# ajzhai/PEANUT

Measured on AMD Instinct MI355X. Metric: maps/sec for 480x480x(4+N_cat) prediction fwd, batch 32, higher is better.
Workload: dtype f32; 1 GPU; 480x480, 14-channel (4+10) partial maps -> 6-class prediction forward (PSPNet R50-V1c-D8), batch 32 per GPU, seeded random-init weights; survey_config=2, global_batch=32, parallelism=dp1 (map shards, no data-path collective)

## Files before the change

peanut_amd/csrc/options.h:

```cpp
#pragma once
#include <stdlib.h>
#include <string.h>

#include <string>

namespace peanut {

enum OptionId {
  OPT_PW_GLDS, OPT_PW256_MINK, OPT_PW256_MINTILES, OPT_PW256_PHASE, OPT_PW256_SKIP_PAD, OPT_PW256W_MINK, OPT_PW256W_MINTILES, OPT_PW256P_MINK, OPT_PW256P_MINTILES, OPT_PW256P_FLUSH, OPT_PW256P_ORDER, OPT_PW256P_STREAMK, OPT_PW256WP_MINK, OPT_PW256WP_MINTILES, OPT_PW256WP_NPRE, OPT_PW256WP_STAGGER, OPT_PW_ARES, OPT_PW_SKINNY,
  OPT_PW_ARES_MINUNITS, OPT_PATCH_MINTILES, OPT_STEM_NCHW, OPT_BN64_MAXK, OPT_PW_BN64_MAXK, OPT_PW64_MAXTILES, OPT_FP32_BK, OPT_NCHUNK, OPT_RES_PREFETCH, OPT_SPLIT_MODEL,
  OPT_RS_CONV, OPT_RS_BN64_MAXK, OPT_RS256_MINK, OPT_RS256_MINTILES, OPT_RS64_MAXK, OPT_RS64_MAXTILES,
  OPT_WINO_M, OPT_WINO_HEAD_M, OPT_WINO6_MAXDIL, OPT_WINO5_MINDIL, OPT_WINO_FLUSH_CH, OPT_WINO_MIN_CIN, OPT_WINO_NARROW_MINPIX, OPT_WINO_SMALL_MAXWG, OPT_DEFER_SPLITK,
  OPT_PPM_OVERLAP, OPT_PPM_GROUPED, OPT_PPM_TERM_ROWS, OPT_PPM_GROUP_ROWS, OPT_RCNN_WINO_M, OPT_RCNN_STEM_S2D, OPT_RCNN_RPN_FUSED, OPT_RCNN_FPN_OVERLAP, OPT_RCNN_RANK_SORT, OPT_RCNN_TOPK_SLICE, OPT_RCNN_NMS_LEVELS, OPT_FMM_LOCAL32, OPT_FMM_MAX_PASSES, OPT_FMM_BLOCKED, OPT_FMM_INNER,
  OPT_DEBUG_POISON_ALLOC,
  OPT_COUNT
};

struct OptionInfo {
  const char* key;
  long long def;
  bool upload_time;
  const char* help;
};

inline const OptionInfo* option_table() {
  static const OptionInfo t[OPT_COUNT] = {
      {"pw_glds", 1, false, "fp32 1x1 convs / grouped GEMMs on the LDS-DMA kernels of conv_pw.hip (0: conv_igemm)"},
      {"pw256_mink", 1024, false, "fewest input channels for the 256 x 128 three-stage kernel"},
      {"pw256_mintiles", 256, false, "fewest 256 x 128 tiles for that kernel"},
      {"pw256_phase", 1, false, "the two waves of a SIMD request their LDS-DMA pieces half an iteration apart"},
      {"pw256_skip_pad", 1, false, "256 x 128 kernel, grouped GEMMs: waves whose rows are all group padding issue no MFMAs (0: compute the zero rows)"},
      {"pw256w_mink", 768, false, "fewest input channels for the 256 x 256 two-stage kernel (0: off)"},
      {"pw256w_mintiles", 1536, false, "fewest 256 x 256 tiles for that kernel"},
      {"pw256p_mink", 512, false, "fewest input channels for the persistent 256 x 128 kernel (conv_pw256p.hip; 0: off)"},
      {"pw256p_mintiles", 512, false, "fewest 256 x 128 tiles for that kernel"},
// ... 10 lines not shown
      {"patch_mintiles", 1024, false, "3x3 convs of 16 / 32 input channels on the persistent LDS-patch kernel (conv_patch.hip) from this many 8 x 16 output tiles (0: off)"},
      {"stem_nchw", 1, false, "prediction forward: the first stem conv reads the NCHW input itself (conv_patch.hip, NCHW variant) instead of a layout pass + NHWC conv (fp32 mode, when the patch kernel takes the layer)"},
      {"bn64_maxk", 256, true, "128 x 64 tiles for layers with at most this many input channels"},
      {"pw_bn64_maxk", 128, true, "pointwise layers / Winograd position GEMMs: weights PACKED 64 wide up to this many input channels (wider layers: 128-wide packing, 64-wide tiles chosen per shape)"},
      {"pw64_maxtiles", 512, false, "a 128-wide-packed pointwise layer with at most bn64_maxk input channels runs 128 x 64 tiles while its 128 x 128 tiling has fewer tiles than this (two per CU)"},
      {"fp32_bk", 0, true, "16: force 16-channel k-tiles in conv_igemm (experiment)"},
      {"nchunk", 8, false, "n-tiles per chunk of the tile order (0: n fastest over all n-tiles)"},
      {"res_prefetch", 1, false, "request the first residual rows before the last k-tile's MFMAs"},
      {"split_model", 1, false, "tail split-K plan counts CUs (1) or resident slots (0)"},
      {"rs_conv", 1, true, "emulated modes: non-pointwise convs on conv_rs.hip (0: fp32 MFMA kernel)"},
      {"rs_bn64_maxk", 128, true, "emulated modes: 128 x 64 tiles up to this many input channels"},
      {"rs256_mink", 512, false, "emulated modes: fewest input channels for the 256 x 256 kernel"},
      {"rs256_mintiles", 256, false, "emulated modes: fewest 256 x 256 tiles for it"},
      {"rs64_maxk", 512, false, "emulated modes: 64 x 64 tiles up to this many input channels"},
      {"rs64_maxtiles", 128, false, "emulated modes: ... and below this many 128-row tiles"},
      {"wino_m", 0, true, "4 / 5 / 6: force one Winograd form on every eligible layer (0: policy)"},
      {"wino_head_m", 0, true, "4 / 5 / 6: Winograd form of the PSP bottleneck (0: policy)"},
      {"wino6_maxdil", 4, true, "largest dilation that gets an F(6x6) form"},
      {"wino5_mindil", 4, true, "smallest dilation that also gets an F(5x5) form (0: none)"},
      {"wino_flush_ch", 64, true, "channels per partial sum of the position GEMMs' two-level accumulation (0: off)"},
      {"wino_min_cin", 0, true, "fewest input channels of a Winograd layer (0: the planner's policy)"},
      {"wino_narrow_minpix", 20000, false, "layers under 128 channels take their Winograd form from this many input pixels on (round 6: 100 000 -> 20 000 -- with the small-problem transforms one 720 x 720 map's layer1 conv2, 32 400 pixels, gains 5 us per layer as F(6x6); profiles/r9e)"},
      {"wino_small_maxwg", 1024, false, "Winograd transforms: launches with fewer workgroups than this of the one-thread-per-tile kernels take the small-problem variants (a workgroup per tile and 64-channel slice, a thread per line, through LDS; bit-identical; 0: never)"},
      {"defer_splitk", 1, false, "a Bottleneck conv1 whose every tile is split along k leaves its partial tiles unsummed and conv2's (small-problem) Winograd input transform sums them: one launch fewer per block at batch 1, bit-identical (0: every conv runs its own reduce); read when a (B, H, W) plan is built"},
      {"ppm_overlap", -1, false, "pyramid branch of the PSP head on a side stream: 0 / 1, -1 = by size"},
      {"ppm_grouped", -1, false, "per-scale PSP GEMMs as one grouped launch: 0 / 1, -1 = by size"},
      {"ppm_term_rows", 1, false, "folded pyramid term: one wave per output row, no barrier in the row loop (0: the workgroup-wide two-phase kernel)"},
      {"ppm_group_rows", 0, false, "pyramid pooling, row pass: rows added up per workgroup (1..5; 0 = by size: as many as still leave ~768 workgroups)"},
      {"rcnn_wino_m", 0, true, "detector front end: 4 / 5 / 6 pins one Winograd form (0: per shape)"},
      {"rcnn_stem_s2d", 1, true, "detector stem 7x7 stride 2 as a space-to-depth 4x4 conv"},
      {"rcnn_rpn_fused", 1, false, "detector: the RPN head on all five pyramid levels as one chain (five input transforms, ONE grouped Winograd GEMM, five output transforms, one objectness and one anchor-delta GEMM over all levels' rows: 12 launches instead of 25); read when a (B, H, W) plan is built"},
      {"rcnn_fpn_overlap", 0, false, "detector: the FPN output convs of p5, p4, p3 on a side stream next to the lateral / top-down chain that ends in p2's (round 5 experiment, bit-identical; measured SLOWER at batch 1, 5.70 against 5.61 ms per frame, profiles/r8: off); read when a (B, H, W) plan is built"},
      {"rcnn_rank_sort", 1, false, "detector: the RPN candidates of an image are ordered by counting the larger keys (n / 64 workgroups) instead of one workgroup's bitonic sort (round 5; same order: the keys are distinct)"},
      {"rcnn_topk_slice", 20480, false, "detector: objectness logits per workgroup of the per-level top-k (a level is cut into up to 8 ranges whose k largest are merged by counting; 0: one workgroup per level, round 4)"},
      {"rcnn_nms_levels", 1, false, "detector: the proposal NMS level by level (five 16 x 16-word suppression blocks and five scans per image side by side, post-NMS top-k by counting) instead of one score-sorted list per image (round 5; same proposals)"},
      {"fmm_local32", 1, false, "goal solver: single-precision local solve inside a tile"},
      {"fmm_max_passes", 24, false, "goal solver: hard ceiling of the second-order ordering passes; they stop as soon as a pass changes nothing (6-10 passes on the agent's 960 x 960 map; peanut_goal_converged reports whether they reached their fixed point)"},
      {"fmm_blocked", 1, false, "goal solver: a wave relaxes its 8 x 8 block of the tile to convergence between workgroup barriers (round 5; 0: one Jacobi sweep of the whole tile per barrier pair)"},
      {"fmm_inner", 48, false, "goal solver: iterations a wave spends on its block before it publishes it (blocked rounds)"},
      {"debug_poison_alloc", 0, false, "test switch: every device allocation the library makes for itself (workspace arenas, conv / Winograd / split-K scratch, the detector's and the goal solver's buffers, the map projection's arrays, uploaded weights before their copy) is filled with 0xFF bytes straight after hipMalloc -- fp32 / fp64 read NaN, int reads -1, 64-bit keys all ones -- so a kernel that reads a slot nothing wrote shows up as a changed result (tests/test_workspace_gpu.py); 0: allocations stay as the allocator returns them, no extra call"},
  };
  return t;
}

struct Options {
  long long v[OPT_COUNT];
// ... 49 lines not shown
```

peanut_amd/csrc/winograd.hip:

```cpp
#include <stdlib.h>

#include <atomic>

#include "common.h"
#include "conv_common.h"

namespace peanut {

namespace {

template <typename V>
__device__ __forceinline__ V fmak(V a, float k, V c) { return __builtin_elementwise_fma(a, (V)k, c); }

__device__ __forceinline__ void bt6(const f32x4 d0, const f32x4 d1, const f32x4 d2, const f32x4 d3, const f32x4 d4,
                                    const f32x4 d5, f32x4& t0, f32x4& t1, f32x4& t2, f32x4& t3, f32x4& t4, f32x4& t5) {
#pragma clang fp contract(off)
  const f32x4 a = fmak(d2, -2.25f, d4), b = fmak(d3, 0.75f, -1.6875f * d1);
  const f32x4 c = fmak(d2, -0.5625f, d4), e = fmak(d3, 1.5f, -0.84375f * d1);
  t0 = fmak(d0, 1.265625f, fmak(d2, -2.8125f, d4));
  t1 = a + b;
  t2 = a - b;
  t3 = c + e;
  t4 = c - e;
  t5 = fmak(d1, 1.265625f, fmak(d3, -2.8125f, d5));
}

__device__ __forceinline__ void at6(const f32x4 m0, const f32x4 m1, const f32x4 m2, const f32x4 m3, const f32x4 m4,
                                    const f32x4 m5, f32x4& y0, f32x4& y1, f32x4& y2, f32x4& y3) {
#pragma clang fp contract(off)
  const f32x4 s12 = m1 + m2, d12 = m1 - m2, s34 = m3 + m4, d34 = m3 - m4;
  y0 = m0 + s12 + s34;
  y1 = fmak(d12, 0.75f, 1.5f * d34);
  y2 = fmak(s12, 0.5625f, 2.25f * s34);
  y3 = fmak(d12, 0.421875f, fmak(d34, 3.375f, m5));
}

struct WinoGeom {
  int B, H, W, C;
  int d, th, tw;
  long long n_tiles, m_pad;
};

__device__ __forceinline__ void decode_tile(const WinoGeom& g, long long t, int& b, int& oy, int& ox, int& ty, int& tx) {
  tx = (int)(t % g.tw); t /= g.tw;
  ty = (int)(t % g.th); t /= g.th;
  ox = (int)(t % g.d); t /= g.d;
  oy = (int)(t % g.d);
  b = (int)(t / g.d);
}

__device__ __forceinline__ bool decode_thread(long long idx, int groups, long long n_tiles, int& cg, long long& tile) {
  cg = (int)(idx % groups);
  tile = idx / groups;
  return tile < n_tiles;
}

__global__ __launch_bounds__(256) void wino_input_kernel(const float* __restrict__ x, float* __restrict__ V, const WinoGeom g) {
  const int groups = g.C >> 2;
  const long long total = g.n_tiles * groups;
  for (long long idx = (long long)blockIdx.x * blockDim.x + threadIdx.x; idx < total;
       idx += (long long)gridDim.x * blockDim.x) {
    int cg;
    long long tile;
    if (!decode_thread(idx, groups, g.n_tiles, cg, tile)) continue;
    int b, oy, ox, ty, tx;
    decode_tile(g, tile, b, oy, ox, ty, tx);
    const int r0 = oy + g.d * (4 * ty - 1), c0 = ox + g.d * (4 * tx - 1);
    const float* xb = x + (size_t)b * g.H * g.W * g.C + cg * 4;
    f32x4 p[6][6];
#pragma unroll
    for (int i = 0; i < 6; ++i) {
      const int r = r0 + i * g.d;
      const bool rok = (unsigned)r < (unsigned)g.H;
#pragma unroll
      for (int j = 0; j < 6; ++j) {
        const int c = c0 + j * g.d;
        f32x4 v = {0.f, 0.f, 0.f, 0.f};
        if (rok && (unsigned)c < (unsigned)g.W) v = *reinterpret_cast<const f32x4*>(xb + ((size_t)r * g.W + c) * g.C);
        p[i][j] = v;
      }
    }
#pragma unroll
    for (int j = 0; j < 6; ++j)
      bt6(p[0][j], p[1][j], p[2][j], p[3][j], p[4][j], p[5][j], p[0][j], p[1][j], p[2][j], p[3][j], p[4][j], p[5][j]);
    float* vb = V + (size_t)tile * g.C + cg * 4;
    const size_t pos_stride = (size_t)g.m_pad * g.C;
#pragma unroll
    for (int i = 0; i < 6; ++i) {
      f32x4 t0, t1, t2, t3, t4, t5;
      bt6(p[i][0], p[i][1], p[i][2], p[i][3], p[i][4], p[i][5], t0, t1, t2, t3, t4, t5);
      float* o = vb + (size_t)(i * 6) * pos_stride;
      *reinterpret_cast<f32x4*>(o) = t0;
      *reinterpret_cast<f32x4*>(o + pos_stride) = t1;
      *reinterpret_cast<f32x4*>(o + 2 * pos_stride) = t2;
      *reinterpret_cast<f32x4*>(o + 3 * pos_stride) = t3;
      *reinterpret_cast<f32x4*>(o + 4 * pos_stride) = t4;
      *reinterpret_cast<f32x4*>(o + 5 * pos_stride) = t5;
    }
  }
}

template <bool RES>
__global__ __launch_bounds__(256) void wino_output_kernel(const float* __restrict__ Mb, const float* __restrict__ scale,
                                                          const float* __restrict__ shift, const float* __restrict__ res,
                                                          float* __restrict__ y, const WinoGeom g, int relu) {
  const int groups = g.C >> 2;
  const long long total = g.n_tiles * groups;
  for (long long idx = (long long)blockIdx.x * blockDim.x + threadIdx.x; idx < total;
       idx += (long long)gridDim.x * blockDim.x) {
    int ng;
    long long tile;
    if (!decode_thread(idx, groups, g.n_tiles, ng, tile)) continue;
    int b, oy, ox, ty, tx;
    decode_tile(g, tile, b, oy, ox, ty, tx);
    const int r0 = oy + g.d * 4 * ty, c0 = ox + g.d * 4 * tx;
    if (r0 >= g.H || c0 >= g.W) continue;
    const float* mb = Mb + (size_t)tile * g.C + ng * 4;
    const size_t pos_stride = (size_t)g.m_pad * g.C;
    f32x4 q[6][4];
#pragma unroll
    for (int i = 0; i < 6; ++i) {
      const float* s = mb + (size_t)(i * 6) * pos_stride;
      const f32x4 m0 = __builtin_nontemporal_load(reinterpret_cast<const f32x4*>(s));
      const f32x4 m1 = __builtin_nontemporal_load(reinterpret_cast<const f32x4*>(s + pos_stride));
      const f32x4 m2 = __builtin_nontemporal_load(reinterpret_cast<const f32x4*>(s + 2 * pos_stride));
      const f32x4 m3 = __builtin_nontemporal_load(reinterpret_cast<const f32x4*>(s + 3 * pos_stride));
      const f32x4 m4 = __builtin_nontemporal_load(reinterpret_cast<const f32x4*>(s + 4 * pos_stride));
      const f32x4 m5 = __builtin_nontemporal_load(reinterpret_cast<const f32x4*>(s + 5 * pos_stride));
      at6(m0, m1, m2, m3, m4, m5, q[i][0], q[i][1], q[i][2], q[i][3]);
    }
    const f32x4 sc = *reinterpret_cast<const f32x4*>(scale + ng * 4);
    const f32x4 sh = *reinterpret_cast<const f32x4*>(shift + ng * 4);
    const size_t img = (size_t)b * g.H * g.W;
    f32x4 rn[4];
    auto res_column = [&](int j, f32x4 (&dst)[4]) __attribute__((always_inline)) {
// ... 16 lines not shown
        if (j + 1 < 4) res_column(j + 1, rn);
      }
      f32x4 o0, o1, o2, o3;
      at6(q[0][j], q[1][j], q[2][j], q[3][j], q[4][j], q[5][j], o0, o1, o2, o3);
      const int c = c0 + j * g.d;
      if (c >= g.W) continue;
      const f32x4 o[4] = {o0, o1, o2, o3};
#pragma unroll
      for (int a = 0; a < 4; ++a) {
        const int r = r0 + a * g.d;
        if (r >= g.H) continue;
        const size_t off = (img + (size_t)r * g.W + c) * g.C + ng * 4;
        f32x4 v = o[a] * sc + sh;
        if constexpr (RES) v += rc[a];
        if (relu) v = relu_keep_nan(v);
        *reinterpret_cast<f32x4*>(y + off) = v;
      }
    }
  }
}

typedef float f32x2 __attribute__((ext_vector_type(2)));

__device__ __forceinline__ void bt8(const f32x2 d0, const f32x2 d1, const f32x2 d2, const f32x2 d3, const f32x2 d4, const f32x2 d5,
                                    const f32x2 d6, const f32x2 d7, f32x2& t0, f32x2& t1, f32x2& t2, f32x2& t3, f32x2& t4,
                                    f32x2& t5, f32x2& t6, f32x2& t7) {
#pragma clang fp contract(off)
  const f32x2 e1 = 4.f * d2 + fmak(d4, -5.f, d6), o1 = 2.f * d1 + fmak(d3, -2.5f, 0.5f * d5);
  const f32x2 e2 = fmak(d4, -4.25f, d2) + d6, o2 = fmak(d3, -4.25f, d1) + d5;
  const f32x2 e3 = 0.25f * d2 + fmak(d4, -1.25f, d6), o3 = 0.5f * d1 + fmak(d3, -2.5f, 2.f * d5);
  const f32x2 r0 = fmak(d2 - d4, 5.25f, d6 - d0), r7 = fmak(d3 - d5, 5.25f, d7 - d1);
  t0 = r0; t1 = e1 + o1; t2 = e1 - o1; t3 = e2 + o2; t4 = e2 - o2; t5 = e3 + o3; t6 = e3 - o3; t7 = r7;
}

__device__ __forceinline__ void at8(const f32x2 m0, const f32x2 m1, const f32x2 m2, const f32x2 m3, const f32x2 m4, const f32x2 m5,
                                    const f32x2 m6, const f32x2 m7, f32x2& y0, f32x2& y1, f32x2& y2, f32x2& y3, f32x2& y4, f32x2& y5) {
#pragma clang fp contract(off)
  const f32x2 s1 = m1 + m2, d1 = m1 - m2, s2 = m3 + m4, d2 = m3 - m4, s3 = m5 + m6, d3 = m5 - m6;
  y0 = m0 + s1 + s2 + s3;
  y1 = 0.5f * d1 + d2 + 2.f * d3;
  y2 = 0.25f * s1 + s2 + 4.f * s3;
  y3 = 0.125f * d1 + d2 + 8.f * d3;
  y4 = 0.0625f * s1 + s2 + 16.f * s3;
  y5 = 0.03125f * d1 + d2 + 32.f * d3 + m7;
}

__global__ __launch_bounds__(256) void wino6_input_kernel(const float* __restrict__ x, float* __restrict__ V, const WinoGeom g) {
  const int groups = g.C >> 1;
  const long long total = g.n_tiles * groups;
  for (long long idx = (long long)blockIdx.x * blockDim.x + threadIdx.x; idx < total;
       idx += (long long)gridDim.x * blockDim.x) {
    int cg;
    long long tile;
    if (!decode_thread(idx, groups, g.n_tiles, cg, tile)) continue;
    int b, oy, ox, ty, tx;
    decode_tile(g, tile, b, oy, ox, ty, tx);
    const int r0 = oy + g.d * (6 * ty - 1), c0 = ox + g.d * (6 * tx - 1);
    const float* xb = x + (size_t)b * g.H * g.W * g.C + cg * 2;
    f32x2 p[8][8];
#pragma unroll
    for (int i = 0; i < 8; ++i) {
      const int r = r0 + i * g.d;
      const bool rok = (unsigned)r < (unsigned)g.H;
#pragma unroll
      for (int j = 0; j < 8; ++j) {
        const int c = c0 + j * g.d;
        f32x2 v = {0.f, 0.f};
        if (rok && (unsigned)c < (unsigned)g.W) v = *reinterpret_cast<const f32x2*>(xb + ((size_t)r * g.W + c) * g.C);
        p[i][j] = v;
      }
    }
#pragma unroll
    for (int j = 0; j < 8; ++j)
      bt8(p[0][j], p[1][j], p[2][j], p[3][j], p[4][j], p[5][j], p[6][j], p[7][j],
          p[0][j], p[1][j], p[2][j], p[3][j], p[4][j], p[5][j], p[6][j], p[7][j]);
    float* vb = V + (size_t)tile * g.C + cg * 2;
    const size_t pos_stride = (size_t)g.m_pad * g.C;
#pragma unroll
    for (int i = 0; i < 8; ++i) {
      f32x2 t[8];
      bt8(p[i][0], p[i][1], p[i][2], p[i][3], p[i][4], p[i][5], p[i][6], p[i][7], t[0], t[1], t[2], t[3], t[4], t[5], t[6], t[7]);
      float* o = vb + (size_t)(i * 8) * pos_stride;
#pragma unroll
      for (int j = 0; j < 8; ++j) *reinterpret_cast<f32x2*>(o + j * pos_stride) = t[j];
    }
  }
}

template <bool RES>
__global__ __launch_bounds__(256) void wino6_output_kernel(const float* __restrict__ Mb, const float* __restrict__ scale,
                                                           const float* __restrict__ shift, const float* __restrict__ res,
                                                           float* __restrict__ y, const WinoGeom g, int relu) {
  const int groups = g.C >> 1;
  const long long total = g.n_tiles * groups;
  for (long long idx = (long long)blockIdx.x * blockDim.x + threadIdx.x; idx < total;
       idx += (long long)gridDim.x * blockDim.x) {
    int ng;
    long long tile;
    if (!decode_thread(idx, groups, g.n_tiles, ng, tile)) continue;
    int b, oy, ox, ty, tx;
    decode_tile(g, tile, b, oy, ox, ty, tx);
    const int r0 = oy + g.d * 6 * ty, c0 = ox + g.d * 6 * tx;
    if (r0 >= g.H || c0 >= g.W) continue;
    const float* mb = Mb + (size_t)tile * g.C + ng * 2;
    const size_t pos_stride = (size_t)g.m_pad * g.C;
    f32x2 q[8][6];
#pragma unroll
    for (int i = 0; i < 8; ++i) {
      const float* s = mb + (size_t)(i * 8) * pos_stride;
      f32x2 m[8];
#pragma unroll
      for (int j = 0; j < 8; ++j) m[j] = __builtin_nontemporal_load(reinterpret_cast<const f32x2*>(s + j * pos_stride));
      at8(m[0], m[1], m[2], m[3], m[4], m[5], m[6], m[7], q[i][0], q[i][1], q[i][2], q[i][3], q[i][4], q[i][5]);
    }
    const f32x2 sc = *reinterpret_cast<const f32x2*>(scale + ng * 2);
    const f32x2 sh = *reinterpret_cast<const f32x2*>(shift + ng * 2);
    const size_t img = (size_t)b * g.H * g.W;
    f32x2 rn[6];
    auto res_column = [&](int j, f32x2 (&dst)[6]) __attribute__((always_inline)) {
      const int c = c0 + j * g.d;
#pragma unroll
      for (int a = 0; a < 6; ++a) {
// ... 7 lines not shown
#pragma unroll
    for (int j = 0; j < 6; ++j) {
      f32x2 rc[6];
      if constexpr (RES) {
#pragma unroll
        for (int a = 0; a < 6; ++a) rc[a] = rn[a];
        if (j + 1 < 6) res_column(j + 1, rn);
      }
      f32x2 o[6];
      at8(q[0][j], q[1][j], q[2][j], q[3][j], q[4][j], q[5][j], q[6][j], q[7][j], o[0], o[1], o[2], o[3], o[4], o[5]);
      const int c = c0 + j * g.d;
      if (c >= g.W) continue;
#pragma unroll
      for (int a = 0; a < 6; ++a) {
        const int r = r0 + a * g.d;
        if (r >= g.H) continue;
        const size_t off = (img + (size_t)r * g.W + c) * g.C + ng * 2;
        f32x2 v = o[a] * sc + sh;
        if constexpr (RES) v += rc[a];
        if (relu) { v.x = relu_keep_nan(v.x); v.y = relu_keep_nan(v.y); }
        *reinterpret_cast<f32x2*>(y + off) = v;
      }
    }
  }
}

__device__ __forceinline__ void bt7(const f32x2 d0, const f32x2 d1, const f32x2 d2, const f32x2 d3, const f32x2 d4, const f32x2 d5,
                                    const f32x2 d6, f32x2& t0, f32x2& t1, f32x2& t2, f32x2& t3, f32x2& t4, f32x2& t5, f32x2& t6) {
  const f32x2 r0 = d5 - 0.75f * d0 + 0.25f * d1 + 3.75f * d2 - 1.25f * d3 - 3.f * d4;
  const f32x2 r1 = d5 + 1.5f * d1 + 2.5f * (d2 - d3 - d4);
  const f32x2 r2 = d5 - 1.5f * d1 + 3.5f * (d2 - d4) + 0.5f * d3;
  const f32x2 r3 = d5 + 0.75f * d1 + 0.5f * d2 - 3.25f * d3 - 2.f * d4;
  const f32x2 r4 = d5 - 0.75f * d1 + d2 + 2.75f * d3 - 4.f * d4;
  const f32x2 r5 = d5 + 0.25f * d1 - 1.25f * d3;
  const f32x2 r6 = d6 - 0.75f * d1 + 0.25f * d2 + 3.75f * d3 - 1.25f * d4 - 3.f * d5;
  t0 = r0; t1 = r1; t2 = r2; t3 = r3; t4 = r4; t5 = r5; t6 = r6;
}

__device__ __forceinline__ void at7(const f32x2 m0, const f32x2 m1, const f32x2 m2, const f32x2 m3, const f32x2 m4, const f32x2 m5,
                                    const f32x2 m6, f32x2& y0, f32x2& y1, f32x2& y2, f32x2& y3, f32x2& y4) {
  const f32x2 s1 = m1 + m2, d1 = m1 - m2, s2 = m3 + m4, d2 = m3 - m4;
  y0 = m0 + s1 + s2 + m5;
  y1 = 0.5f * d1 + d2 + 3.f * m5;
  y2 = 0.25f * s1 + s2 + 9.f * m5;
  y3 = 0.125f * d1 + d2 + 27.f * m5;
  y4 = 0.0625f * s1 + s2 + 81.f * m5 + m6;
}

__global__ __launch_bounds__(256) void wino5_input_kernel(const float* __restrict__ x, float* __restrict__ V, const WinoGeom g) {
  const int groups = g.C >> 1;
  const long long total = g.n_tiles * groups;
  for (long long idx = (long long)blockIdx.x * blockDim.x + threadIdx.x; idx < total;
       idx += (long long)gridDim.x * blockDim.x) {
    int cg;
    long long tile;
    if (!decode_thread(idx, groups, g.n_tiles, cg, tile)) continue;
    int b, oy, ox, ty, tx;
    decode_tile(g, tile, b, oy, ox, ty, tx);
    const int r0 = oy + g.d * (5 * ty - 1), c0 = ox + g.d * (5 * tx - 1);
    const float* xb = x + (size_t)b * g.H * g.W * g.C + cg * 2;
    f32x2 p[7][7];
#pragma unroll
    for (int i = 0; i < 7; ++i) {
      const int r = r0 + i * g.d;
      const bool rok = (unsigned)r < (unsigned)g.H;
#pragma unroll
      for (int j = 0; j < 7; ++j) {
        const int c = c0 + j * g.d;
        f32x2 v = {0.f, 0.f};
        if (rok && (unsigned)c < (unsigned)g.W) v = *reinterpret_cast<const f32x2*>(xb + ((size_t)r * g.W + c) * g.C);
        p[i][j] = v;
      }
    }
#pragma unroll
    for (int j = 0; j < 7; ++j)
      bt7(p[0][j], p[1][j], p[2][j], p[3][j], p[4][j], p[5][j], p[6][j],
          p[0][j], p[1][j], p[2][j], p[3][j], p[4][j], p[5][j], p[6][j]);
    float* vb = V + (size_t)tile * g.C + cg * 2;
    const size_t pos_stride = (size_t)g.m_pad * g.C;
#pragma unroll
    for (int i = 0; i < 7; ++i) {
      f32x2 t[7];
      bt7(p[i][0], p[i][1], p[i][2], p[i][3], p[i][4], p[i][5], p[i][6], t[0], t[1], t[2], t[3], t[4], t[5], t[6]);
      float* o = vb + (size_t)(i * 7) * pos_stride;
#pragma unroll
      for (int j = 0; j < 7; ++j) *reinterpret_cast<f32x2*>(o + j * pos_stride) = t[j];
    }
  }
}

__global__ __launch_bounds__(256) void wino5_output_kernel(const float* __restrict__ Mb, const float* __restrict__ scale,
                                                           const float* __restrict__ shift, const float* __restrict__ res,
                                                           float* __restrict__ y, const WinoGeom g, int relu) {
  const int groups = g.C >> 1;
  const long long total = g.n_tiles * groups;
  for (long long idx = (long long)blockIdx.x * blockDim.x + threadIdx.x; idx < total;
       idx += (long long)gridDim.x * blockDim.x) {
    int ng;
    long long tile;
    if (!decode_thread(idx, groups, g.n_tiles, ng, tile)) continue;
    int b, oy, ox, ty, tx;
    decode_tile(g, tile, b, oy, ox, ty, tx);
    const int r0 = oy + g.d * 5 * ty, c0 = ox + g.d * 5 * tx;
    if (r0 >= g.H || c0 >= g.W) continue;
    const float* mb = Mb + (size_t)tile * g.C + ng * 2;
    const size_t pos_stride = (size_t)g.m_pad * g.C;
    f32x2 q[7][5];
#pragma unroll
    for (int i = 0; i < 7; ++i) {
      const float* s = mb + (size_t)(i * 7) * pos_stride;
      f32x2 m[7];
#pragma unroll
      for (int j = 0; j < 7; ++j) m[j] = __builtin_nontemporal_load(reinterpret_cast<const f32x2*>(s + j * pos_stride));
      at7(m[0], m[1], m[2], m[3], m[4], m[5], m[6], q[i][0], q[i][1], q[i][2], q[i][3], q[i][4]);
    }
    const f32x2 sc = *reinterpret_cast<const f32x2*>(scale + ng * 2);
    const f32x2 sh = *reinterpret_cast<const f32x2*>(shift + ng * 2);
    const size_t img = (size_t)b * g.H * g.W;
#pragma unroll
    for (int j = 0; j < 5; ++j) {
      f32x2 o[5];
      at7(q[0][j], q[1][j], q[2][j], q[3][j], q[4][j], q[5][j], q[6][j], o[0], o[1], o[2], o[3], o[4]);
      const int c = c0 + j * g.d;
// ... 270 lines not shown
    f32x4 v = o[k] * sc + sh;
    if constexpr (RES) v += rc[k];
    if (relu) v = relu_keep_nan(v);
    *reinterpret_cast<f32x4*>(y + off) = v;
  }
}

int wino_small_lanes(long long n_tiles, int C, int m) {
  const long long maxwg = opt(OPT_WINO_SMALL_MAXWG);
  if (maxwg <= 0 || (m != 4 && m != 6)) return 0;
  const long long big_wgs = (n_tiles * (m == 4 ? C / 4 : C / 2) + 255) / 256;
  if (big_wgs >= maxwg) return 0;
  const int per32 = m == 4 ? 128 : 64, per16 = per32 / 2;
  const int lanes = C % per32 == 0 ? 32 : (C % per16 == 0 ? 16 : 0);
  if (!lanes || n_tiles * (C / (lanes * (m == 4 ? 4 : 2))) > 0x7fffffffLL) return 0;
  return lanes;
}

int grid_for(long long total) {
  long long blocks = (total + 255) / 256;
  if (blocks > 256LL * 64) blocks = 256LL * 64;
  if (blocks < 1) blocks = 1;
  return (int)blocks;
}

}

void wino_geometry(int B, int H, int W, int dil, int* th, int* tw, long long* n_tiles, long long* m_pad, int gran, int m) {
  const int hs = (H + dil - 1) / dil, wsub = (W + dil - 1) / dil;
  *th = (hs + m - 1) / m;
  *tw = (wsub + m - 1) / m;
  *n_tiles = (long long)B * dil * dil * *th * *tw;
  *m_pad = (*n_tiles + gran - 1) / gran * gran;
}

void wino_transform_weights(const float* w_oihw, int cout, int cin, float* out, int m) {
  static const double G4[6][3] = {{64.0 / 81, 0, 0},
                                  {-128.0 / 243, -32.0 / 81, -8.0 / 27},
                                  {-128.0 / 243, 32.0 / 81, -8.0 / 27},
                                  {32.0 / 243, 16.0 / 81, 8.0 / 27},
                                  {32.0 / 243, -16.0 / 81, 8.0 / 27},
                                  {0, 0, 1}};
  static const double G6[8][3] = {{-1, 0, 0},
                                  {32.0 / 45, 16.0 / 45, 8.0 / 45},
                                  {32.0 / 45, -16.0 / 45, 8.0 / 45},
                                  {-2.0 / 9, -2.0 / 9, -2.0 / 9},
// ... 44 lines not shown
  const long long total = g.n_tiles * (m == 4 ? C / 4 : C / 2);
  const bool defer = df && df->valid;
  DeferredSrc src{};
  if (defer) {
    if (df->cout != C || (long long)df->M != (long long)B * H * W || !wino_small_lanes(g.n_tiles, C, m))
      return fail(-2, "wino_input: deferred split-K partials do not match this transform");
    src = DeferredSrc{df->partial, df->scale, df->shift, df->alpha, df->split_p, df->ntiles, df->relu};
    g_deferred_count.fetch_add(1, std::memory_order_relaxed);
  }
  if (const int lanes = wino_small_lanes(g.n_tiles, C, m)) {
    const unsigned grid = (unsigned)(g.n_tiles * (C / (lanes * (m == 4 ? 4 : 2))));
#define PEANUT_WINO_SMALL_IN(K, L, T)                                                                          \
    do {                                                                                                       \
      if (defer && src.split_p == 4) hipLaunchKernelGGL((K<L, 4>), dim3(grid), dim3(T), 0, s, x, V, g, src);   \
      else if (defer && src.split_p == 2) hipLaunchKernelGGL((K<L, 2>), dim3(grid), dim3(T), 0, s, x, V, g, src); \
      else if (defer) hipLaunchKernelGGL((K<L, 0>), dim3(grid), dim3(T), 0, s, x, V, g, src);                  \
      else hipLaunchKernelGGL((K<L, -1>), dim3(grid), dim3(T), 0, s, x, V, g, src);                            \
    } while (0)
    if (m == 6 && lanes == 32) PEANUT_WINO_SMALL_IN(wino6_input_small_kernel, 32, 256);
    else if (m == 6) PEANUT_WINO_SMALL_IN(wino6_input_small_kernel, 16, 128);
    else if (lanes == 32) PEANUT_WINO_SMALL_IN(wino4_input_small_kernel, 32, 192);
    else PEANUT_WINO_SMALL_IN(wino4_input_small_kernel, 16, 96);
#undef PEANUT_WINO_SMALL_IN
  } else if (m == 6) hipLaunchKernelGGL(wino6_input_kernel, dim3(grid_for(total)), dim3(256), 0, s, x, V, g);
  else if (m == 5) hipLaunchKernelGGL(wino5_input_kernel, dim3(grid_for(total)), dim3(256), 0, s, x, V, g);
  else hipLaunchKernelGGL(wino_input_kernel, dim3(grid_for(total)), dim3(256), 0, s, x, V, g);
  hipError_t e = hipGetLastError();
  if (e != hipSuccess) return fail(-3, std::string("wino_input launch: ") + hipGetErrorString(e));
  return 0;
}

int launch_wino_output(const float* Mb, const float* scale, const float* shift, const float* res, float* y,
                       int B, int H, int W, int C, int dil, int relu, hipStream_t s, int gran, int m, long long m_pad_total) {
  if (C % 4 || m < 4 || m > 6) return fail(-2, "wino_output: channels must be a multiple of 4, tiles 4x4, 5x5 or 6x6");
  WinoGeom g{B, H, W, C, dil, 0, 0, 0, 0};
  wino_geometry(B, H, W, dil, &g.th, &g.tw, &g.n_tiles, &g.m_pad, gran, m);
  if (m_pad_total > 0) g.m_pad = m_pad_total;
  const long long total = g.n_tiles * (m == 4 ? C / 4 : C / 2);
  if (const int lanes = wino_small_lanes(g.n_tiles, C, m)) {
    const unsigned grid = (unsigned)(g.n_tiles * (C / (lanes * (m == 4 ? 4 : 2))));
#define PEANUT_WINO_SMALL_OUT(K, R, L, T) hipLaunchKernelGGL((K<R, L>), dim3(grid), dim3(T), 0, s, Mb, scale, shift, res, y, g, relu)
    if (m == 6 && lanes == 32) { if (res) PEANUT_WINO_SMALL_OUT(wino6_output_small_kernel, true, 32, 256); else PEANUT_WINO_SMALL_OUT(wino6_output_small_kernel, false, 32, 256); }
    else if (m == 6) { if (res) PEANUT_WINO_SMALL_OUT(wino6_output_small_kernel, true, 16, 128); else PEANUT_WINO_SMALL_OUT(wino6_output_small_kernel, false, 16, 128); }
    else if (lanes == 32) { if (res) PEANUT_WINO_SMALL_OUT(wino4_output_small_kernel, true, 32, 192); else PEANUT_WINO_SMALL_OUT(wino4_output_small_kernel, false, 32, 192); }
    else { if (res) PEANUT_WINO_SMALL_OUT(wino4_output_small_kernel, true, 16, 96); else PEANUT_WINO_SMALL_OUT(wino4_output_small_kernel, false, 16, 96); }
#undef PEANUT_WINO_SMALL_OUT
  } else if (m == 6 && res) hipLaunchKernelGGL(wino6_output_kernel<true>, dim3(grid_for(total)), dim3(256), 0, s, Mb, scale, shift, res, y, g, relu);
  else if (m == 6) hipLaunchKernelGGL(wino6_output_kernel<false>, dim3(grid_for(total)), dim3(256), 0, s, Mb, scale, shift, res, y, g, relu);
  else if (m == 5) hipLaunchKernelGGL(wino5_output_kernel, dim3(grid_for(total)), dim3(256), 0, s, Mb, scale, shift, res, y, g, relu);
  else if (res) hipLaunchKernelGGL(wino_output_kernel<true>, dim3(grid_for(total)), dim3(256), 0, s, Mb, scale, shift, res, y, g, relu);
  else hipLaunchKernelGGL(wino_output_kernel<false>, dim3(grid_for(total)), dim3(256), 0, s, Mb, scale, shift, res, y, g, relu);
  hipError_t e = hipGetLastError();
  if (e != hipSuccess) return fail(-3, std::string("wino_output launch: ") + hipGetErrorString(e));
  return 0;
}

}
```

Before: 887.2 maps/s.

## Add LDS two-stage F(6x6) Winograd transforms and XCD-local tile ordering

Adds workgroup-per-run-of-tiles F(6x6) input and output transform kernels. They do separable row and column passes through LDS with 16-byte accesses and replace the one-thread-per-tile kernels for large layers without a residual. Input transforms of F(6x6) and F(5x5) also switch to an XCD-local tile order when a tile row fits the L2, so a tile's halo is fetched across the fabric once. The aim is fewer redundant and uncoalesced global reads in the transforms, at the cost of more kernel variants, an added barrier, and LDS occupancy limits.

```diff
diff --git a/peanut_amd/csrc/options.h b/peanut_amd/csrc/options.h
--- a/peanut_amd/csrc/options.h
+++ b/peanut_amd/csrc/options.h
@@ -10,7 +10,7 @@
   OPT_PW_GLDS, OPT_PW256_MINK, OPT_PW256_MINTILES, OPT_PW256_PHASE, OPT_PW256_SKIP_PAD, OPT_PW256W_MINK, OPT_PW256W_MINTILES, OPT_PW256P_MINK, OPT_PW256P_MINTILES, OPT_PW256P_FLUSH, OPT_PW256P_ORDER, OPT_PW256P_STREAMK, OPT_PW256WP_MINK, OPT_PW256WP_MINTILES, OPT_PW256WP_NPRE, OPT_PW256WP_STAGGER, OPT_PW_ARES, OPT_PW_SKINNY,
   OPT_PW_ARES_MINUNITS, OPT_PATCH_MINTILES, OPT_STEM_NCHW, OPT_BN64_MAXK, OPT_PW_BN64_MAXK, OPT_PW64_MAXTILES, OPT_FP32_BK, OPT_NCHUNK, OPT_RES_PREFETCH, OPT_SPLIT_MODEL,
   OPT_RS_CONV, OPT_RS_BN64_MAXK, OPT_RS256_MINK, OPT_RS256_MINTILES, OPT_RS64_MAXK, OPT_RS64_MAXTILES,
-  OPT_WINO_M, OPT_WINO_HEAD_M, OPT_WINO6_MAXDIL, OPT_WINO5_MINDIL, OPT_WINO_FLUSH_CH, OPT_WINO_MIN_CIN, OPT_WINO_NARROW_MINPIX, OPT_WINO_SMALL_MAXWG, OPT_DEFER_SPLITK,
+  OPT_WINO_M, OPT_WINO_HEAD_M, OPT_WINO6_MAXDIL, OPT_WINO5_MINDIL, OPT_WINO_FLUSH_CH, OPT_WINO_MIN_CIN, OPT_WINO_NARROW_MINPIX, OPT_WINO_SMALL_MAXWG, OPT_WINO_XFORM, OPT_DEFER_SPLITK,
   OPT_PPM_OVERLAP, OPT_PPM_GROUPED, OPT_PPM_TERM_ROWS, OPT_PPM_GROUP_ROWS, OPT_RCNN_WINO_M, OPT_RCNN_STEM_S2D, OPT_RCNN_RPN_FUSED, OPT_RCNN_FPN_OVERLAP, OPT_RCNN_RANK_SORT, OPT_RCNN_TOPK_SLICE, OPT_RCNN_NMS_LEVELS, OPT_FMM_LOCAL32, OPT_FMM_MAX_PASSES, OPT_FMM_BLOCKED, OPT_FMM_INNER,
   OPT_DEBUG_POISON_ALLOC,
   OPT_COUNT
@@ -67,6 +67,7 @@
       {"wino_min_cin", 0, true, "fewest input channels of a Winograd layer (0: the planner's policy)"},
       {"wino_narrow_minpix", 20000, false, "layers under 128 channels take their Winograd form from this many input pixels on (round 6: 100 000 -> 20 000 -- with the small-problem transforms one 720 x 720 map's layer1 conv2, 32 400 pixels, gains 5 us per layer as F(6x6); profiles/r9e)"},
       {"wino_small_maxwg", 1024, false, "Winograd transforms: launches with fewer workgroups than this of the one-thread-per-tile kernels take the small-problem variants (a workgroup per tile and 64-channel slice, a thread per line, through LDS; bit-identical; 0: never)"},
+      {"wino_xform", 1, false, "large-problem Winograd transforms: 1 = F(6x6) on the two-stage kernels (a workgroup per run of adjacent tiles and channel slice, a thread per line, through LDS, 16-byte accesses; layers with a residual keep the one-thread-per-tile kernel) and the F(6x6) / F(5x5) input transforms in XCD-local tile order where a tile row fits the L2 (the workgroups that share an L2 take one contiguous eighth of the tiles, so a tile's halo crosses the fabric once); 2 = the one-thread-per-tile kernels of every form in XCD-local order; 0 = those kernels in linear order.  Bit-identical"},
       {"defer_splitk", 1, false, "a Bottleneck conv1 whose every tile is split along k leaves its partial tiles unsummed and conv2's (small-problem) Winograd input transform sums them: one launch fewer per block at batch 1, bit-identical (0: every conv runs its own reduce); read when a (B, H, W) plan is built"},
       {"ppm_overlap", -1, false, "pyramid branch of the PSP head on a side stream: 0 / 1, -1 = by size"},
       {"ppm_grouped", -1, false, "per-scale PSP GEMMs as one grouped launch: 0 / 1, -1 = by size"},
diff --git a/peanut_amd/csrc/winograd.hip b/peanut_amd/csrc/winograd.hip
--- a/peanut_amd/csrc/winograd.hip
+++ b/peanut_amd/csrc/winograd.hip
@@ -39,6 +39,7 @@
   int B, H, W, C;
   int d, th, tw;
   long long n_tiles, m_pad;
+  int xcd;
 };
 
 __device__ __forceinline__ void decode_tile(const WinoGeom& g, long long t, int& b, int& oy, int& ox, int& ty, int& tx) {
@@ -49,20 +50,33 @@
   b = (int)(t / g.d);
 }
 
-__device__ __forceinline__ bool decode_thread(long long idx, int groups, long long n_tiles, int& cg, long long& tile) {
-  cg = (int)(idx % groups);
-  tile = idx / groups;
-  return tile < n_tiles;
-}
-
+
+__host__ __device__ __forceinline__ void xcd_tile_range(long long n_tiles, int x, long long& lo, long long& hi) {
+  lo = n_tiles * x / 8;
+  hi = n_tiles * (x + 1) / 8;
+}
+
+struct WorkIter {
+  long long first, end, step, tile0;
+};
+template <bool XCD>
+__device__ __forceinline__ WorkIter work_items(const WinoGeom& g, int groups) {
+  if constexpr (!XCD) {
+    return WorkIter{(long long)blockIdx.x * blockDim.x + threadIdx.x, g.n_tiles * groups, (long long)gridDim.x * blockDim.x, 0};
+  } else {
+    long long lo, hi;
+    xcd_tile_range(g.n_tiles, blockIdx.x & 7, lo, hi);
+    return WorkIter{(long long)(blockIdx.x >> 3) * blockDim.x + threadIdx.x, (hi - lo) * groups, (long long)(gridDim.x >> 3) * blockDim.x, lo};
+  }
+}
+
+template <bool XCD>
 __global__ __launch_bounds__(256) void wino_input_kernel(const float* __restrict__ x, float* __restrict__ V, const WinoGeom g) {
   const int groups = g.C >> 2;
-  const long long total = g.n_tiles * groups;
-  for (long long idx = (long long)blockIdx.x * blockDim.x + threadIdx.x; idx < total;
-       idx += (long long)gridDim.x * blockDim.x) {
-    int cg;
-    long long tile;
-    if (!decode_thread(idx, groups, g.n_tiles, cg, tile)) continue;
+  const WorkIter it = work_items<XCD>(g, groups);
+  for (long long idx = it.first; idx < it.end; idx += it.step) {
+    const int cg = (int)(idx % groups);
+    const long long tile = it.tile0 + idx / groups;
     int b, oy, ox, ty, tx;
     decode_tile(g, tile, b, oy, ox, ty, tx);
     const int r0 = oy + g.d * (4 * ty - 1), c0 = ox + g.d * (4 * tx - 1);
@@ -100,17 +114,15 @@
   }
 }
 
-template <bool RES>
+template <bool RES, bool XCD>
 __global__ __launch_bounds__(256) void wino_output_kernel(const float* __restrict__ Mb, const float* __restrict__ scale,
                                                           const float* __restrict__ shift, const float* __restrict__ res,
                                                           float* __restrict__ y, const WinoGeom g, int relu) {
   const int groups = g.C >> 2;
-  const long long total = g.n_tiles * groups;
-  for (long long idx = (long long)blockIdx.x * blockDim.x + threadIdx.x; idx < total;
-       idx += (long long)gridDim.x * blockDim.x) {
-    int ng;
-    long long tile;
-    if (!decode_thread(idx, groups, g.n_tiles, ng, tile)) continue;
+  const WorkIter it = work_items<XCD>(g, groups);
+  for (long long idx = it.first; idx < it.end; idx += it.step) {
+    const int ng = (int)(idx % groups);
+    const long long tile = it.tile0 + idx / groups;
     int b, oy, ox, ty, tx;
     decode_tile(g, tile, b, oy, ox, ty, tx);
     const int r0 = oy + g.d * 4 * ty, c0 = ox + g.d * 4 * tx;
@@ -173,21 +185,23 @@
 
 typedef float f32x2 __attribute__((ext_vector_type(2)));
 
-__device__ __forceinline__ void bt8(const f32x2 d0, const f32x2 d1, const f32x2 d2, const f32x2 d3, const f32x2 d4, const f32x2 d5,
-                                    const f32x2 d6, const f32x2 d7, f32x2& t0, f32x2& t1, f32x2& t2, f32x2& t3, f32x2& t4,
-                                    f32x2& t5, f32x2& t6, f32x2& t7) {
+template <typename V>
+__device__ __forceinline__ void bt8(const V d0, const V d1, const V d2, const V d3, const V d4, const V d5,
+                                    const V d6, const V d7, V& t0, V& t1, V& t2, V& t3, V& t4,
+                                    V& t5, V& t6, V& t7) {
 #pragma clang fp contract(off)
-  const f32x2 e1 = 4.f * d2 + fmak(d4, -5.f, d6), o1 = 2.f * d1 + fmak(d3, -2.5f, 0.5f * d5);
-  const f32x2 e2 = fmak(d4, -4.25f, d2) + d6, o2 = fmak(d3, -4.25f, d1) + d5;
-  const f32x2 e3 = 0.25f * d2 + fmak(d4, -1.25f, d6), o3 = 0.5f * d1 + fmak(d3, -2.5f, 2.f * d5);
-  const f32x2 r0 = fmak(d2 - d4, 5.25f, d6 - d0), r7 = fmak(d3 - d5, 5.25f, d7 - d1);
+  const V e1 = 4.f * d2 + fmak(d4, -5.f, d6), o1 = 2.f * d1 + fmak(d3, -2.5f, 0.5f * d5);
+  const V e2 = fmak(d4, -4.25f, d2) + d6, o2 = fmak(d3, -4.25f, d1) + d5;
+  const V e3 = 0.25f * d2 + fmak(d4, -1.25f, d6), o3 = 0.5f * d1 + fmak(d3, -2.5f, 2.f * d5);
+  const V r0 = fmak(d2 - d4, 5.25f, d6 - d0), r7 = fmak(d3 - d5, 5.25f, d7 - d1);
   t0 = r0; t1 = e1 + o1; t2 = e1 - o1; t3 = e2 + o2; t4 = e2 - o2; t5 = e3 + o3; t6 = e3 - o3; t7 = r7;
 }
 
-__device__ __forceinline__ void at8(const f32x2 m0, const f32x2 m1, const f32x2 m2, const f32x2 m3, const f32x2 m4, const f32x2 m5,
-                                    const f32x2 m6, const f32x2 m7, f32x2& y0, f32x2& y1, f32x2& y2, f32x2& y3, f32x2& y4, f32x2& y5) {
+template <typename V>
+__device__ __forceinline__ void at8(const V m0, const V m1, const V m2, const V m3, const V m4, const V m5,
+                                    const V m6, const V m7, V& y0, V& y1, V& y2, V& y3, V& y4, V& y5) {
 #pragma clang fp contract(off)
-  const f32x2 s1 = m1 + m2, d1 = m1 - m2, s2 = m3 + m4, d2 = m3 - m4, s3 = m5 + m6, d3 = m5 - m6;
+  const V s1 = m1 + m2, d1 = m1 - m2, s2 = m3 + m4, d2 = m3 - m4, s3 = m5 + m6, d3 = m5 - m6;
   y0 = m0 + s1 + s2 + s3;
   y1 = 0.5f * d1 + d2 + 2.f * d3;
   y2 = 0.25f * s1 + s2 + 4.f * s3;
@@ -196,14 +210,13 @@
   y5 = 0.03125f * d1 + d2 + 32.f * d3 + m7;
 }
 
+template <bool XCD>
 __global__ __launch_bounds__(256) void wino6_input_kernel(const float* __restrict__ x, float* __restrict__ V, const WinoGeom g) {
   const int groups = g.C >> 1;
-  const long long total = g.n_tiles * groups;
-  for (long long idx = (long long)blockIdx.x * blockDim.x + threadIdx.x; idx < total;
-       idx += (long long)gridDim.x * blockDim.x) {
-    int cg;
-    long long tile;
-    if (!decode_thread(idx, groups, g.n_tiles, cg, tile)) continue;
+  const WorkIter it = work_items<XCD>(g, groups);
+  for (long long idx = it.first; idx < it.end; idx += it.step) {
+    const int cg = (int)(idx % groups);
+    const long long tile = it.tile0 + idx / groups;
     int b, oy, ox, ty, tx;
     decode_tile(g, tile, b, oy, ox, ty, tx);
     const int r0 = oy + g.d * (6 * ty - 1), c0 = ox + g.d * (6 * tx - 1);
@@ -238,17 +251,15 @@
   }
 }
 
-template <bool RES>
+template <bool RES, bool XCD>
 __global__ __launch_bounds__(256) void wino6_output_kernel(const float* __restrict__ Mb, const float* __restrict__ scale,
                                                            const float* __restrict__ shift, const float* __restrict__ res,
                                                            float* __restrict__ y, const WinoGeom g, int relu) {
   const int groups = g.C >> 1;
-  const long long total = g.n_tiles * groups;
-  for (long long idx = (long long)blockIdx.x * blockDim.x + threadIdx.x; idx < total;
-       idx += (long long)gridDim.x * blockDim.x) {
-    int ng;
-    long long tile;
-    if (!decode_thread(idx, groups, g.n_tiles, ng, tile)) continue;
+  const WorkIter it = work_items<XCD>(g, groups);
+  for (long long idx = it.first; idx < it.end; idx += it.step) {
+    const int ng = (int)(idx % groups);
+    const long long tile = it.tile0 + idx / groups;
     int b, oy, ox, ty, tx;
     decode_tile(g, tile, b, oy, ox, ty, tx);
     const int r0 = oy + g.d * 6 * ty, c0 = ox + g.d * 6 * tx;
@@ -302,6 +313,125 @@
         *reinterpret_cast<f32x2*>(y + off) = v;
       }
     }
+  }
+}
+
+struct RunUnit {
+  long long tile0;
+  int nt;
+  int slice;
+};
+__host__ __device__ __forceinline__ long long run_of_tile(long long t, int tw, int rpr, int R) { return t / tw * rpr + (int)(t % tw) / R; }
+__host__ __device__ __forceinline__ long long xcd_run_units(long long n_tiles, int tw, int R, int slices, int x, long long& run_lo, long long& lo, long long& hi) {
+  xcd_tile_range(n_tiles, x, lo, hi);
+  if (hi <= lo) return 0;
+  const int rpr = (tw + R - 1) / R;
+  run_lo = run_of_tile(lo, tw, rpr, R);
+  return (run_of_tile(hi - 1, tw, rpr, R) - run_lo + 1) * slices;
+}
+__device__ __forceinline__ bool run_unit(const WinoGeom& g, int R, int slices, RunUnit& w) {
+  long long run_lo = 0, lo, hi, units, u;
+  if (g.xcd) {
+    units = xcd_run_units(g.n_tiles, g.tw, R, slices, blockIdx.x & 7, run_lo, lo, hi);
+    u = blockIdx.x >> 3;
+  } else {
+    lo = 0; hi = g.n_tiles; u = blockIdx.x;
+    units = (run_of_tile(hi - 1, g.tw, (g.tw + R - 1) / R, R) + 1) * slices;
+  }
+  if (u >= units) return false;
+  const int rpr = (g.tw + R - 1) / R;
+  const long long run = run_lo + u / slices, row = run / rpr;
+  long long ta = row * g.tw + (run % rpr) * R, tb = ta + R;
+  if (tb > (row + 1) * g.tw) tb = (row + 1) * g.tw;
+  if (ta < lo) ta = lo;
+  if (tb > hi) tb = hi;
+  w.tile0 = ta;
+  w.nt = (int)(tb - ta);
+  w.slice = (int)(u % slices);
+  return true;
+}
+
+template <int R, int L>
+__global__ __launch_bounds__(8 * R * L) void wino6_input_lds_kernel(const float* __restrict__ x, float* __restrict__ V, const WinoGeom g) {
+  constexpr int NCOL = 6 * R + 2;
+  __shared__ f32x4 u[8][NCOL][L];
+  RunUnit w;
+  if (!run_unit(g, R, g.C / (4 * L), w)) return;
+  const int l = threadIdx.x % L, a = threadIdx.x / L;
+  const int cg = w.slice * L + l;
+  int b, oy, ox, ty, tx;
+  decode_tile(g, w.tile0, b, oy, ox, ty, tx);
+  if (a < 6 * w.nt + 2) {
+    const int r0 = oy + g.d * (6 * ty - 1), c = ox + g.d * (6 * tx - 1 + a);
+    const bool cok = (unsigned)c < (unsigned)g.W;
+    const float* xb = x + (size_t)b * g.H * g.W * g.C + cg * 4;
+    f32x4 p[8];
+#pragma unroll
+    for (int i = 0; i < 8; ++i) {
+      const int r = r0 + i * g.d;
+      f32x4 v = {0.f, 0.f, 0.f, 0.f};
+      if (cok && (unsigned)r < (unsigned)g.H) v = *reinterpret_cast<const f32x4*>(xb + ((size_t)r * g.W + c) * g.C);
+      p[i] = v;
+    }
+    bt8(p[0], p[1], p[2], p[3], p[4], p[5], p[6], p[7], p[0], p[1], p[2], p[3], p[4], p[5], p[6], p[7]);
+#pragma unroll
+    for (int i = 0; i < 8; ++i) u[i][a][l] = p[i];
+  }
+  __syncthreads();
+  const int r = a >> 3, i = a & 7;
+  if (r >= w.nt) return;
+  f32x4 q[8], t[8];
+#pragma unroll
+  for (int j = 0; j < 8; ++j) q[j] = u[i][6 * r + j][l];
+  bt8(q[0], q[1], q[2], q[3], q[4], q[5], q[6], q[7], t[0], t[1], t[2], t[3], t[4], t[5], t[6], t[7]);
+  const size_t pos_stride = (size_t)g.m_pad * g.C;
+  float* o = V + (size_t)(w.tile0 + r) * g.C + cg * 4 + (size_t)(i * 8) * pos_stride;
+#pragma unroll
+  for (int j = 0; j < 8; ++j) *reinterpret_cast<f32x4*>(o + j * pos_stride) = t[j];
+}
+
+template <int R, int L>
+__global__ __launch_bounds__(8 * R * L) void wino6_output_lds_kernel(const float* __restrict__ Mb, const float* __restrict__ scale,
+                                                                    const float* __restrict__ shift, float* __restrict__ y,
+                                                                    const WinoGeom g, int relu) {
+  __shared__ f32x4 qs[R][8][6][L];
+  RunUnit w;
+  if (!run_unit(g, R, g.C / (4 * L), w)) return;
+  const int l = threadIdx.x % L, a = threadIdx.x / L;
+  const int r = a >> 3, i = a & 7;
+  const int ng = w.slice * L + l;
+  int b, oy, ox, ty, tx;
+  decode_tile(g, w.tile0, b, oy, ox, ty, tx);
+  const int r0 = oy + g.d * 6 * ty, c0 = ox + g.d * 6 * (tx + r);
+  if (r0 >= g.H) return;
+  const bool live = r < w.nt && c0 < g.W;
+  const size_t pos_stride = (size_t)g.m_pad * g.C;
+  const int c = c0 + i * g.d;
+  const size_t img = (size_t)b * g.H * g.W;
+  if (live) {
+    const float* sp = Mb + (size_t)(w.tile0 + r) * g.C + ng * 4 + (size_t)(i * 8) * pos_stride;
+    f32x4 m[8], q[6];
+#pragma unroll
+    for (int j = 0; j < 8; ++j) m[j] = __builtin_nontemporal_load(reinterpret_cast<const f32x4*>(sp + j * pos_stride));
+    at8(m[0], m[1], m[2], m[3], m[4], m[5], m[6], m[7], q[0], q[1], q[2], q[3], q[4], q[5]);
+#pragma unroll
+    for (int j = 0; j < 6; ++j) qs[r][i][j][l] = q[j];
+  }
+  __syncthreads();
+  if (!live || i >= 6 || c >= g.W) return;
+  const f32x4 sc = *reinterpret_cast<const f32x4*>(scale + ng * 4);
+  const f32x4 sh = *reinterpret_cast<const f32x4*>(shift + ng * 4);
+  f32x4 o[6];
+  at8(qs[r][0][i][l], qs[r][1][i][l], qs[r][2][i][l], qs[r][3][i][l], qs[r][4][i][l], qs[r][5][i][l], qs[r][6][i][l], qs[r][7][i][l],
+      o[0], o[1], o[2], o[3], o[4], o[5]);
+#pragma unroll
+  for (int k = 0; k < 6; ++k) {
+    const int rr = r0 + k * g.d;
+    if (rr >= g.H) continue;
+    const size_t off = (img + (size_t)rr * g.W + c) * g.C + ng * 4;
+    f32x4 v = o[k] * sc + sh;
+    if (relu) v = relu_keep_nan(v);
+    *reinterpret_cast<f32x4*>(y + off) = v;
   }
 }
 
@@ -327,14 +457,13 @@
   y4 = 0.0625f * s1 + s2 + 81.f * m5 + m6;
 }
 
+template <bool XCD>
 __global__ __launch_bounds__(256) void wino5_input_kernel(const float* __restrict__ x, float* __restrict__ V, const WinoGeom g) {
   const int groups = g.C >> 1;
-  const long long total = g.n_tiles * groups;
-  for (long long idx = (long long)blockIdx.x * blockDim.x + threadIdx.x; idx < total;
-       idx += (long long)gridDim.x * blockDim.x) {
-    int cg;
-    long long tile;
-    if (!decode_thread(idx, groups, g.n_tiles, cg, tile)) continue;
+  const WorkIter it = work_items<XCD>(g, groups);
+  for (long long idx = it.first; idx < it.end; idx += it.step) {
+    const int cg = (int)(idx % groups);
+    const long long tile = it.tile0 + idx / groups;
     int b, oy, ox, ty, tx;
     decode_tile(g, tile, b, oy, ox, ty, tx);
     const int r0 = oy + g.d * (5 * ty - 1), c0 = ox + g.d * (5 * tx - 1);
@@ -369,16 +498,15 @@
   }
 }
 
+template <bool XCD>
 __global__ __launch_bounds__(256) void wino5_output_kernel(const float* __restrict__ Mb, const float* __restrict__ scale,
                                                            const float* __restrict__ shift, const float* __restrict__ res,
                                                            float* __restrict__ y, const WinoGeom g, int relu) {
   const int groups = g.C >> 1;
-  const long long total = g.n_tiles * groups;
-  for (long long idx = (long long)blockIdx.x * blockDim.x + threadIdx.x; idx < total;
-       idx += (long long)gridDim.x * blockDim.x) {
-    int ng;
-    long long tile;
-    if (!decode_thread(idx, groups, g.n_tiles, ng, tile)) continue;
+  const WorkIter it = work_items<XCD>(g, groups);
+  for (long long idx = it.first; idx < it.end; idx += it.step) {
+    const int ng = (int)(idx % groups);
+    const long long tile = it.tile0 + idx / groups;
     int b, oy, ox, ty, tx;
     decode_tile(g, tile, b, oy, ox, ty, tx);
     const int r0 = oy + g.d * 5 * ty, c0 = ox + g.d * 5 * tx;
@@ -695,6 +823,31 @@
   if (blocks > 256LL * 64) blocks = 256LL * 64;
   if (blocks < 1) blocks = 1;
   return (int)blocks;
+}
+
+int grid_for_xcd(long long n_tiles, int groups) {
+  long long per_xcd = ((n_tiles + 7) / 8 * groups + 255) / 256;
+  if (per_xcd > (1LL << 21)) per_xcd = 1LL << 21;
+  if (per_xcd < 1) per_xcd = 1;
+  return (int)(8 * per_xcd);
+}
+
+long long wino6_lds_grid(const WinoGeom& g, int R, int L) {
+  if (g.C % (4 * L) != 0) return 0;
+  long long most = 0;
+  if (!g.xcd) return (run_of_tile(g.n_tiles - 1, g.tw, (g.tw + R - 1) / R, R) + 1) * (g.C / (4 * L));
+  for (int x = 0; x < 8; ++x) {
+    long long run_lo, lo, hi;
+    const long long units = xcd_run_units(g.n_tiles, g.tw, R, g.C / (4 * L), x, run_lo, lo, hi);
+    if (units > most) most = units;
+  }
+  return most > 0 && most * 8 <= 0x7fffffffLL ? most * 8 : 0;
+}
+inline int wino6_lds_lanes(int C) { return C % 128 == 0 ? 32 : (C % 64 == 0 ? 16 : 0); }
+
+inline bool wino_rows_fit_l2(const WinoGeom& g, int m) {
+  const double row_bytes = (double)g.tw * m * m * g.C * 4.0 * (1.0 + (double)((m + 2) * (m + 2)) / (m * m));
+  return row_bytes <= 2.0 * 1024 * 1024;
 }
 
 }
@@ -785,9 +938,22 @@
     else if (lanes == 32) PEANUT_WINO_SMALL_IN(wino4_input_small_kernel, 32, 192);
     else PEANUT_WINO_SMALL_IN(wino4_input_small_kernel, 16, 96);
 #undef PEANUT_WINO_SMALL_IN
-  } else if (m == 6) hipLaunchKernelGGL(wino6_input_kernel, dim3(grid_for(total)), dim3(256), 0, s, x, V, g);
-  else if (m == 5) hipLaunchKernelGGL(wino5_input_kernel, dim3(grid_for(total)), dim3(256), 0, s, x, V, g);
-  else hipLaunchKernelGGL(wino_input_kernel, dim3(grid_for(total)), dim3(256), 0, s, x, V, g);
+  } else {
+    const long long xform = opt(OPT_WINO_XFORM);
+    const int groups = m == 4 ? C / 4 : C / 2;
+    const int L = (xform == 1 && m == 6) ? wino6_lds_lanes(C) : 0;
+    g.xcd = xform == 2 || (xform == 1 && (L || m == 5) && wino_rows_fit_l2(g, m));
+    const int grid = g.xcd ? grid_for_xcd(g.n_tiles, groups) : grid_for(total);
+    const long long lds_grid = L ? wino6_lds_grid(g, 32 / L, L) : 0;
+    if (lds_grid && L == 32) hipLaunchKernelGGL((wino6_input_lds_kernel<1, 32>), dim3((unsigned)lds_grid), dim3(256), 0, s, x, V, g);
+    else if (lds_grid) hipLaunchKernelGGL((wino6_input_lds_kernel<2, 16>), dim3((unsigned)lds_grid), dim3(256), 0, s, x, V, g);
+    else if (m == 6 && g.xcd) hipLaunchKernelGGL(wino6_input_kernel<true>, dim3(grid), dim3(256), 0, s, x, V, g);
+    else if (m == 6) hipLaunchKernelGGL(wino6_input_kernel<false>, dim3(grid), dim3(256), 0, s, x, V, g);
+    else if (m == 5 && g.xcd) hipLaunchKernelGGL(wino5_input_kernel<true>, dim3(grid), dim3(256), 0, s, x, V, g);
+    else if (m == 5) hipLaunchKernelGGL(wino5_input_kernel<false>, dim3(grid), dim3(256), 0, s, x, V, g);
+    else if (g.xcd) hipLaunchKernelGGL(wino_input_kernel<true>, dim3(grid), dim3(256), 0, s, x, V, g);
+    else hipLaunchKernelGGL(wino_input_kernel<false>, dim3(grid), dim3(256), 0, s, x, V, g);
+  }
   hipError_t e = hipGetLastError();
   if (e != hipSuccess) return fail(-3, std::string("wino_input launch: ") + hipGetErrorString(e));
   return 0;
@@ -808,11 +974,23 @@
     else if (lanes == 32) { if (res) PEANUT_WINO_SMALL_OUT(wino4_output_small_kernel, true, 32, 192); else PEANUT_WINO_SMALL_OUT(wino4_output_small_kernel, false, 32, 192); }
     else { if (res) PEANUT_WINO_SMALL_OUT(wino4_output_small_kernel, true, 16, 96); else PEANUT_WINO_SMALL_OUT(wino4_output_small_kernel, false, 16, 96); }
 #undef PEANUT_WINO_SMALL_OUT
-  } else if (m == 6 && res) hipLaunchKernelGGL(wino6_output_kernel<true>, dim3(grid_for(total)), dim3(256), 0, s, Mb, scale, shift, res, y, g, relu);
-  else if (m == 6) hipLaunchKernelGGL(wino6_output_kernel<false>, dim3(grid_for(total)), dim3(256), 0, s, Mb, scale, shift, res, y, g, relu);
-  else if (m == 5) hipLaunchKernelGGL(wino5_output_kernel, dim3(grid_for(total)), dim3(256), 0, s, Mb, scale, shift, res, y, g, relu);
-  else if (res) hipLaunchKernelGGL(wino_output_kernel<true>, dim3(grid_for(total)), dim3(256), 0, s, Mb, scale, shift, res, y, g, relu);
-  else hipLaunchKernelGGL(wino_output_kernel<false>, dim3(grid_for(total)), dim3(256), 0, s, Mb, scale, shift, res, y, g, relu);
+  } else {
+    const long long xform = opt(OPT_WINO_XFORM);
+    const int groups = m == 4 ? C / 4 : C / 2;
+    const int L = (xform == 1 && m == 6 && !res) ? wino6_lds_lanes(C) : 0;
+    g.xcd = xform == 2;
+    const int grid = g.xcd ? grid_for_xcd(g.n_tiles, groups) : grid_for(total);
+    const long long lds_grid = L ? wino6_lds_grid(g, 32 / L, L) : 0;
+    if (lds_grid && L == 32) hipLaunchKernelGGL((wino6_output_lds_kernel<1, 32>), dim3((unsigned)lds_grid), dim3(256), 0, s, Mb, scale, shift, y, g, relu);
+    else if (lds_grid) hipLaunchKernelGGL((wino6_output_lds_kernel<2, 16>), dim3((unsigned)lds_grid), dim3(256), 0, s, Mb, scale, shift, y, g, relu);
+#define PEANUT_WINO_OUT(K, ...) hipLaunchKernelGGL((K<__VA_ARGS__>), dim3(grid), dim3(256), 0, s, Mb, scale, shift, res, y, g, relu)
+    else if (m == 6 && res) { if (g.xcd) PEANUT_WINO_OUT(wino6_output_kernel, true, true); else PEANUT_WINO_OUT(wino6_output_kernel, true, false); }
+    else if (m == 6) { if (g.xcd) PEANUT_WINO_OUT(wino6_output_kernel, false, true); else PEANUT_WINO_OUT(wino6_output_kernel, false, false); }
+    else if (m == 5) { if (g.xcd) PEANUT_WINO_OUT(wino5_output_kernel, true); else PEANUT_WINO_OUT(wino5_output_kernel, false); }
+    else if (res) { if (g.xcd) PEANUT_WINO_OUT(wino_output_kernel, true, true); else PEANUT_WINO_OUT(wino_output_kernel, true, false); }
+    else { if (g.xcd) PEANUT_WINO_OUT(wino_output_kernel, false, true); else PEANUT_WINO_OUT(wino_output_kernel, false, false); }
+#undef PEANUT_WINO_OUT
+  }
   hipError_t e = hipGetLastError();
   if (e != hipSuccess) return fail(-3, std::string("wino_output launch: ") + hipGetErrorString(e));
   return 0;
```

Result: no change. 890.3 maps/s, median of 6 (+0.4%).
